# imazen/imageflow

Hardware: AMD Instinct MI355X
Metric: megapixels/sec resize (4K->200px Robidoux) (higher is better)
Workload: dtype f32; 1 GPU; BASELINE cfg2: 256 frames (256 on rank 0) 3840x2160 BGRA8 -> 200x200 Robidoux, linear light, ReplaceSelf, alpha not meaningful, device resident, pattern=mixed; frames_per_gpu=256, total_frames=256, kernel=fused_resample_kernel, gather=none, gather_mode=none, reserved_cus_while_gathering=0, rccl_ranks=1, backend=none

## Files before the change

### imageflow_amd/csrc/api.cpp

```cpp
#include <hip/hip_runtime.h>

#include <algorithm>
#include <cstdio>
#include <cstring>
#include <map>
#include <memory>
#include <mutex>
#include <tuple>
#include <vector>

#include "hip_entry.hpp"
#include "resample_plan.hpp"

namespace ifhip {
hipError_t launch_fused(const ResampleArgs& a, int slots, bool alpha, bool per_pixel, uint32_t grid, uint32_t block,
                        size_t lds, hipStream_t st);
hipError_t launch_generic(const ResampleArgs& a, bool alpha, float4* scratch, uint32_t img0, uint32_t n_img,
                          hipStream_t st);
hipError_t launch_banded(const ResampleArgs& a, bool alpha, const BandedArgs& b, uint32_t grid_x, size_t lds, hipStream_t st);
hipError_t launch_apply_matte(uint8_t* d_bgra, size_t image_bytes, uint32_t n_images, uint32_t w, uint32_t h,
                              uint32_t stride, uint32_t matte, float mb, float mg, float mr, float ma,
                              const float* s2l, const uint8_t* l2s, hipStream_t st);
}

using namespace ifhip;

namespace {
struct DeviceTables {
    float* s2l = nullptr;
    float* s2f = nullptr;
    uint8_t* l2s = nullptr;
    uint16_t* l2s_thr = nullptr;
};
std::mutex g_dev_mu;
std::map<int, DeviceTables> g_dev_tables;

int device_tables(DeviceTables* out) {
    int dev = -1;
    if (hipGetDevice(&dev) != hipSuccess || dev < 0)
        return fail(IFHIP_GPU_UNAVAILABLE, "GpuUnavailable: no HIP device (hipGetDevice failed); this library has no CPU path");
    std::lock_guard<std::mutex> lk(g_dev_mu);
    auto it = g_dev_tables.find(dev);
    if (it == g_dev_tables.end()) {
        hipDeviceProp_t prop;
        HIP_TRY(hipGetDeviceProperties(&prop, dev));
        if (std::strncmp(prop.gcnArchName, "gfx950", 6) != 0)
            return fail(IFHIP_GPU_UNAVAILABLE, "GpuUnavailable: device %d is %s, this library is built for gfx950 only", dev, prop.gcnArchName);
        const ColorTables& t = color_tables();
        DeviceTables d;
        HIP_TRY(hipMalloc(reinterpret_cast<void**>(&d.s2l), sizeof t.s2l));
        HIP_TRY(hipMalloc(reinterpret_cast<void**>(&d.s2f), sizeof t.s2f));
        HIP_TRY(hipMalloc(reinterpret_cast<void**>(&d.l2s), sizeof t.l2s));
        HIP_TRY(hipMemcpy(d.s2l, t.s2l, sizeof t.s2l, hipMemcpyHostToDevice));
        HIP_TRY(hipMemcpy(d.s2f, t.s2f, sizeof t.s2f, hipMemcpyHostToDevice));
        HIP_TRY(hipMemcpy(d.l2s, t.l2s, sizeof t.l2s, hipMemcpyHostToDevice));
        HIP_TRY(hipMalloc(reinterpret_cast<void**>(&d.l2s_thr), sizeof t.l2s_thr));
        HIP_TRY(hipMemcpy(d.l2s_thr, t.l2s_thr, sizeof t.l2s_thr, hipMemcpyHostToDevice));
        it = g_dev_tables.emplace(dev, d).first;
    }
    *out = it->second;
    return IFHIP_OK;
}

template <typename T>
int upload(const std::vector<T>& v, T** out) {
    *out = nullptr;
    if (v.empty()) return IFHIP_OK;
    HIP_TRY(DEV_MALLOC(out, v.size() * sizeof(T)));
    HIP_TRY(static_cast<hipError_t>(copy_to_device(*out, v.data(), v.size() * sizeof(T))));
    return IFHIP_OK;
}

}

struct ifhip_resample_plan {
    int device = -1;
    PlanTables t;
    uint32_t *d_v_left = nullptr, *d_v_count = nullptr, *d_v_off = nullptr;
    uint32_t *d_h_left = nullptr, *d_h_count = nullptr, *d_h_off = nullptr;
    float *d_v_w = nullptr, *d_h_w = nullptr, *d_h_wu = nullptr, *d_h_wg = nullptr, *d_h_wg2 = nullptr;
    uint4* d_h_meta = nullptr;
    uint32_t *d_h_meta2 = nullptr, *d_h_meta3 = nullptr;
    Strip* d_strips[2] = {nullptr, nullptr};

    ~ifhip_resample_plan() {
        for (void* p : {(void*)d_v_left, (void*)d_v_count, (void*)d_v_off, (void*)d_h_left, (void*)d_h_count,
                        (void*)d_h_off, (void*)d_v_w, (void*)d_h_w, (void*)d_h_wu, (void*)d_h_meta, (void*)d_h_wg, (void*)d_h_meta2, (void*)d_h_wg2, (void*)d_h_meta3, (void*)d_strips[0],
                        (void*)d_strips[1]})
            if (p) (void)DEV_FREE(p);
        for (auto& kv : t.schedules) {
            if (kv.second.d_steps) (void)DEV_FREE(kv.second.d_steps);
            if (kv.second.d_band_begin) (void)DEV_FREE(kv.second.d_band_begin);
        }
    }
};

namespace {

bool trace_launch() { return debug_switch("trace_launch") != nullptr; }

int schedule_on_device(const PlanTables& t, PlannedSchedule* s) {
    std::lock_guard<std::mutex> lk(t.mu);
    if (s->d_steps) return IFHIP_OK;
    VStep* steps = nullptr;
    int rc = upload(s->host.steps, &steps);
    if (rc) return rc;
    rc = upload(s->host.band_begin, &s->d_band_begin);
    if (rc) { (void)DEV_FREE(steps); return rc; }
    s->d_steps = steps;
    return IFHIP_OK;
}

int validate_render(uint32_t in_w, uint32_t in_h, uint32_t in_stride, uint32_t cw, uint32_t ch, uint32_t c_stride,
                    uint32_t x, uint32_t y, uint32_t w, uint32_t h, int working_space, int compositing, uint32_t in_px_bytes = 4) {
    if (static_cast<uint64_t>(h) + y > ch || static_cast<uint64_t>(w) + x > cw)
        return fail(IFHIP_INVALID_ARGUMENT, "InvalidArgument: Destination rectangle for scale2d is out of bounds");
    if (w == 0 || h == 0 || in_w == 0 || in_h == 0)
        return fail(IFHIP_INVALID_ARGUMENT, "InvalidArgument: Bitmap dimensions cannot be zero");
    if (static_cast<uint64_t>(in_w) * in_px_bytes > in_stride || static_cast<uint64_t>(cw) * 4u > c_stride)
        return fail(IFHIP_INVALID_ARGUMENT, "InvalidArgument: stride smaller than a BGRA row");
    if (c_stride & 3u)
        return fail(IFHIP_INVALID_ARGUMENT, "InvalidArgument: canvas stride must be a multiple of 4 bytes");
    if (working_space != IFHIP_SPACE_SRGB && working_space != IFHIP_SPACE_LINEAR)
        return fail(IFHIP_METHOD_NOT_IMPLEMENTED, "MethodNotImplemented: working floatspace %d", working_space);
    if (compositing < IFHIP_REPLACE_SELF || compositing > IFHIP_BLEND_WITH_MATTE)
        return fail(IFHIP_INVALID_ARGUMENT, "InvalidArgument: compositing mode %d", compositing);
    return IFHIP_OK;
}

int enqueue_batch(const ifhip_resample_plan* p, const uint8_t* d_in, size_t in_image_bytes, uint32_t in_stride,
                  int alpha, uint32_t n_images, uint8_t* d_canvas, size_t canvas_image_bytes, uint32_t cw, uint32_t ch,
                  uint32_t c_stride, uint32_t x, uint32_t y, int working_space, int compositing, uint32_t matte,
                  float* d_f32, int force_kernel, hipStream_t st, const uint8_t* d_cb = nullptr, const uint8_t* d_cr = nullptr,
                  bool probe = false) {
    if (!p) return fail(IFHIP_INVALID_ARGUMENT, "InvalidArgument: null plan");
    const PlanTables& t = p->t;
    const bool ycc = d_cb != nullptr;
    int rc = validate_render(t.in_w, t.in_h, in_stride, cw, ch, c_stride, x, y, t.out_w, t.out_h, working_space, compositing, ycc ? 1u : 4u);
    if (rc) return rc;
    if (n_images == 0) return IFHIP_OK;
    if (!d_in || !d_canvas || (ycc && !d_cr)) return fail(IFHIP_INVALID_ARGUMENT, "InvalidArgument: null bitmap pointer");
    if ((reinterpret_cast<uintptr_t>(d_canvas) & 3u) || (canvas_image_bytes & 3u))
        return fail(IFHIP_INVALID_ARGUMENT, "InvalidArgument: canvas pixels must be 4-byte aligned");
    int dev = -1;
    HIP_TRY(hipGetDevice(&dev));
    if (dev != p->device) return fail(IFHIP_INVALID_STATE, "InvalidState: plan belongs to device %d, current device is %d", p->device, dev);
    DeviceTables tb;
    rc = device_tables(&tb);
    if (rc) return rc;

    LaunchInputs in = launch_inputs_now();
    in.alpha = alpha; in.ycc = ycc; in.n_images = n_images; in.in_image_bytes = in_image_bytes; in.in_stride = in_stride;
    in.src_low_bits = (reinterpret_cast<uintptr_t>(d_in) | reinterpret_cast<uintptr_t>(d_cb) | reinterpret_cast<uintptr_t>(d_cr)) & 15u;
    in.force_kernel = force_kernel; in.working_space = working_space; in.probe = probe;
    const LaunchChoice c = choose_launch(t, in);
    if (c.status) return c.status;
    if (trace_launch()) std::fprintf(stderr, "%s\n", format_launch(t, in, c).c_str());
    if (probe) return IFHIP_OK;

    const ColorTables& host_tb = color_tables();
    ResampleArgs a;
    std::memset(&a, 0, sizeof a);
    a.in = d_in; a.in_image_bytes = in_image_bytes; a.in_stride = in_stride; a.in_w = t.in_w; a.in_h = t.in_h;
    a.in_cb = d_cb; a.in_cr = d_cr; a.ycc = ycc ? 1u : 0u;
    a.canvas = d_canvas; a.canvas_image_bytes = canvas_image_bytes; a.c_stride = c_stride; a.x = x; a.y = y;
    a.out_w = t.out_w; a.out_h = t.out_h; a.f32_dump = d_f32;
    a.h_meta = p->d_h_meta; a.h_wu = p->d_h_wu; a.h_wu_floats = static_cast<uint32_t>(t.wu.size());
    a.h_left = p->d_h_left; a.h_count = p->d_h_count;
    a.v_left = p->d_v_left; a.v_count = p->d_v_count; a.v_off = p->d_v_off; a.v_w = p->d_v_w;
    a.h_off = p->d_h_off; a.h_w = p->d_h_w;
    a.linear = working_space == IFHIP_SPACE_LINEAR;
    a.lut_in = a.linear ? tb.s2l : tb.s2f;
    a.l2s = tb.l2s;
    a.l2s_thr = tb.l2s_thr;
    a.mode = compositing;
    const float* s2 = a.linear ? host_tb.s2l : host_tb.s2f;
    a.m0 = s2[matte & 255u]; a.m1 = s2[(matte >> 8) & 255u]; a.m2 = s2[(matte >> 16) & 255u];
    a.matte_a = static_cast<float>(matte >> 24) * (1.0f / 255.0f);
    a.n_images = n_images;

    if (c.kernel == LaunchKernel::Banded) {
        HIP_TRY(launch_banded(a, alpha != 0, c.banded, c.grid, c.lds, st));
        return IFHIP_OK;
    }
    if (c.kernel == LaunchKernel::Fused) {
        if ((rc = schedule_on_device(t, c.schedule))) return rc;
        a.steps = c.schedule->d_steps; a.band_begin = c.schedule->d_band_begin; a.n_bands = c.n_bands;
        a.strips = p->d_strips[alpha ? 1 : 0]; a.n_strips = c.n_strips;
        a.h_groups = c.two_col ? 16u + c.fast_groups : c.fast_groups;
        if (c.two_col) { a.h_wu = p->d_h_wg2; a.h_wu_floats = static_cast<uint32_t>(t.wg2.size()); a.h_meta2 = p->d_h_meta3; }
        else if (c.fast_groups) { a.h_wu = p->d_h_wg; a.h_wu_floats = static_cast<uint32_t>(t.wg.size()); a.h_meta2 = p->d_h_meta2; }
        a.lut_copies_log2 = c.lut_copies_log2;
        a.h_w_in_lds = c.w_in_lds ? 1u : 0u;
        a.l2s_in_lds = c.l2s_in_lds ? 1u : 0u;
        a.frames_per_wg = c.frames_per_wg;
        a.lanes_per_frame = c.lanes_per_frame;
        HIP_TRY(launch_fused(a, t.slots, alpha != 0, c.per_pixel, c.grid, c.lanes_per_frame * c.frames_per_wg, c.lds, st));
        return IFHIP_OK;
    }
    const size_t per_image = static_cast<size_t>(t.out_h) * t.in_w * sizeof(float4);
    float4* scratch = nullptr;
    HIP_TRY(static_cast<hipError_t>(cached_malloc_for_stream(reinterpret_cast<void**>(&scratch), per_image * c.chunk, st, true)));
    hipError_t le = hipSuccess;
    for (uint32_t i0 = 0; i0 < n_images && le == hipSuccess; i0 += c.chunk) {
        const uint32_t n = std::min(c.chunk, n_images - i0);
        le = launch_generic(a, alpha != 0, scratch, i0, n, st);
    }
    const hipError_t fe = static_cast<hipError_t>(cached_free_after(scratch, st));
    HIP_TRY(le);
    HIP_TRY(fe);
    return IFHIP_OK;
}
}

namespace ifhip {
int resample_from_ycc_planes_v(const ifhip_resample_plan* plan, const uint8_t* d_y, const uint8_t* d_cb, const uint8_t* d_cr,
                             size_t plane_bytes, uint32_t pitch, uint32_t n_images, uint8_t* d_canvas, size_t canvas_image_bytes,
                             uint32_t cw, uint32_t ch, uint32_t c_stride, uint32_t x, uint32_t y, int working_space, int compositing,
                             uint32_t matte, void* hip_stream, bool probe) {
    return enqueue_batch(plan, d_y, plane_bytes, pitch, 0, n_images, d_canvas, canvas_image_bytes, cw, ch, c_stride, x, y,
                         working_space, compositing, matte, nullptr, -1, static_cast<hipStream_t>(hip_stream), d_cb, d_cr, probe);
}
void resample_plan_shape(const ifhip_resample_plan* plan, uint32_t* in_w, uint32_t* in_h, uint32_t* out_w, uint32_t* out_h) {
    *in_w = plan->t.in_w; *in_h = plan->t.in_h; *out_w = plan->t.out_w; *out_h = plan->t.out_h;
}
int device_color_tables(const float** s2l, const uint8_t** l2s) {
    DeviceTables tb;
    const int rc = device_tables(&tb);
    if (rc) return rc;
    *s2l = tb.s2l; *l2s = tb.l2s;
    return IFHIP_OK;
}

namespace {
struct PlanKey {
    int device; uint32_t in_w, in_h, w, h; int filter; uint32_t sharpen_bits;
    bool operator<(const PlanKey& o) const {
        return std::tie(device, in_w, in_h, w, h, filter, sharpen_bits) < std::tie(o.device, o.in_w, o.in_h, o.w, o.h, o.filter, o.sharpen_bits);
    }
};
std::mutex g_plan_mu;
typedef std::map<PlanKey, std::pair<std::shared_ptr<ifhip_resample_plan>, uint64_t>> PlanMap;
PlanMap& plan_map() { static PlanMap* m = new PlanMap; return *m; }
uint64_t g_plan_clock = 0;
constexpr size_t kPlanCacheMax = 256;
}
int cached_plan(uint32_t in_w, uint32_t in_h, uint32_t w, uint32_t h, int filter, float sharpen, std::shared_ptr<ifhip_resample_plan>* out) {
    int dev = -1;
    if (hipGetDevice(&dev) != hipSuccess || dev < 0)
        return fail(IFHIP_GPU_UNAVAILABLE, "GpuUnavailable: no HIP device (hipGetDevice failed); this library has no CPU path");
    uint32_t bits;
    std::memcpy(&bits, &sharpen, 4);
    const PlanKey key{dev, in_w, in_h, w, h, filter, bits};
    {
        std::lock_guard<std::mutex> lk(g_plan_mu);
        auto it = plan_map().find(key);
        if (it != plan_map().end()) { it->second.second = ++g_plan_clock; *out = it->second.first; return IFHIP_OK; }
    }
    ifhip_resample_plan* raw = nullptr;
    const int rc = ifhip_resample_plan_create(&raw, in_w, in_h, w, h, filter, sharpen);
    if (rc) return rc;
    std::shared_ptr<ifhip_resample_plan> sp(raw, [](ifhip_resample_plan* q) {
        if (hipStream_t st = static_cast<hipStream_t>(thread_stream()); st && hipStreamQuery(st) != hipSuccess) (void)wait_stream(st);
        (void)hipGetLastError();
        ifhip_resample_plan_destroy(q);
    });
    std::shared_ptr<ifhip_resample_plan> evicted;
    {
        std::lock_guard<std::mutex> lk(g_plan_mu);
        PlanMap& plans = plan_map();
// ... 307 lines not shown
```

### imageflow_amd/csrc/common.hpp

```cpp
#pragma once
#include <cstdint>
#include <memory>
#include <string>
#include <vector>

#include "../../include/imageflow_hip.h"

namespace ifhip {

int fail(int status, const char* fmt, ...) __attribute__((format(printf, 2, 3)));
const char* last_error();

int cached_malloc(void** out, size_t bytes);
int cached_free(void* p);
int cached_malloc_for_stream(void** out, size_t bytes, void* stream, bool for_stream);
int cached_free_after(void* p, void* stream);
int cached_host_malloc(void** out, size_t bytes);
int cached_host_free(void* p);
void quiesced_enter();
void quiesced_leave();
struct QuiescedScope { QuiescedScope() { quiesced_enter(); } ~QuiescedScope() { quiesced_leave(); } };
void* thread_stream();
int wait_stream(void* hip_stream);
int copy_to_device(void* dst, const void* src, size_t bytes);
int stage_to_device(void* dst, const void* src, size_t bytes, void** pin_out);
int copy_to_host(void* dst, const void* src, size_t bytes);
int zero_device(void* dst, size_t bytes);
int require_gfx950(int* device_out);
#define DEV_MALLOC(pp, n) static_cast<hipError_t>(::ifhip::cached_malloc(reinterpret_cast<void**>(pp), (n)))
#define DEV_FREE(p) static_cast<hipError_t>(::ifhip::cached_free(p))

bool icc_describes_srgb(const uint8_t* profile, size_t profile_bytes);
int jpeg_icc_profile(const uint8_t* jpeg, size_t len, int* kind, std::vector<uint8_t>* profile);

const char* debug_switch(const char* key);
inline bool debug_on(const char* key) { return debug_switch(key) != nullptr; }

enum class KernelShape : uint8_t { FlexCubic, CubicFast, Sinc, Box, Triangle, SincWindowed, Jinc, Ginseng };

struct FilterSpec {
    double window = 2.0;
    double blur = 1.0;
    double p1 = 0, p2 = 1, p3 = 1, q1 = 0, q2 = 1, q3 = 1, q4 = 1;
    KernelShape shape = KernelShape::Box;
    int lobe_mode = IFHIP_LOBE_NATURAL;
    float lobe_value = 0.f;

    double eval(double x) const;
    double natural_negative_ratio() const;
};

bool filter_spec_for(int filter, FilterSpec* out);

struct AxisWeights {
    uint32_t n_out = 0, n_in = 0;
    std::vector<uint32_t> left;
    std::vector<uint32_t> count;
    std::vector<uint32_t> offset;
    std::vector<float> w;
    uint32_t max_taps = 0;
};

int build_axis_weights(const FilterSpec& spec, uint32_t out_size, uint32_t in_size, AxisWeights* out);

struct ColorTables {
    float s2l[256];
    float s2f[256];
    uint8_t l2s[16384];
    uint16_t l2s_thr[256];
};
const ColorTables& color_tables();
int device_color_tables(const float** s2l, const uint8_t** l2s);

constexpr int kMaxSlots = 8;
struct alignas(64) VStep {
    int32_t y;
    uint32_t active;
    int32_t flush_slot;
    int32_t out_row;
    float w[kMaxSlots];
    int32_t y_ahead;
    int32_t pad[3];
};
static_assert(sizeof(VStep) == 64, "VStep must be one 64-byte scalar-load line");

struct VSchedule {
    int slots = 0;
    std::vector<VStep> steps;
    std::vector<uint32_t> band_begin;
};
bool build_vschedule(const AxisWeights& wv, int n_bands, int group, int ahead, VSchedule* out);

constexpr int kNotFusable = -1000;
int resample_from_ycc_planes_v(const ifhip_resample_plan* plan, const uint8_t* d_y, const uint8_t* d_cb, const uint8_t* d_cr,
                               size_t plane_bytes, uint32_t pitch, uint32_t n_images, uint8_t* d_canvas, size_t canvas_image_bytes,
                               uint32_t cw, uint32_t ch, uint32_t c_stride, uint32_t x, uint32_t y, int working_space, int compositing,
                               uint32_t matte, void* hip_stream, bool probe = false);
void resample_plan_shape(const ifhip_resample_plan* plan, uint32_t* in_w, uint32_t* in_h, uint32_t* out_w, uint32_t* out_h);
int max_live_rows(const AxisWeights& wv);
int cached_plan(uint32_t in_w, uint32_t in_h, uint32_t w, uint32_t h, int filter, float sharpen, std::shared_ptr<ifhip_resample_plan>* out);

}
```

### imageflow_amd/csrc/resample_fused.hip

```cpp
#include <atomic>
#include <type_traits>

#include "resample_device.hpp"

#ifndef IFHIP_FUSED_K
#error "compile with -DIFHIP_FUSED_K=<ring size 1..8>"
#endif
namespace ifhip {

template <int K, bool ALPHA, bool WLDS, bool PERPIXEL, int FG = 0, bool YCC = false>
__global__ void __launch_bounds__(fused_max_threads(K, ALPHA ? 4 : 3))
__attribute__((amdgpu_waves_per_eu(fused_max_threads(K, ALPHA ? 4 : 3) / 256, fused_max_threads(K, ALPHA ? 4 : 3) / 256)))
fused_resample_kernel(const ResampleArgs a, const VStep* __restrict__ steps) {
    static_assert(FG == 0 || (WLDS && PERPIXEL), "the fast horizontal pass keeps its weights in LDS and maps one lane per pixel");
    constexpr bool TWO = FG >= 16;
    static_assert(!TWO || (!ALPHA && !YCC), "two-column groups: three channels from a BGRA source");
    static_assert(!YCC || (!ALPHA && fused_shape(K, 3).px == 4), "planar source: three channels, four pixels per lane");
    constexpr int C = ALPHA ? 4 : 3;
    constexpr int D = fused_shape(K, C).rows_in_flight;
    constexpr bool PIPE = fused_shape(K, C).pipelined != 0;
    extern __shared__ __attribute__((aligned(16))) unsigned char smem[];

    const uint32_t wtid = threadIdx.x;
    const uint32_t WT = blockDim.x;
    const uint32_t T = a.lanes_per_frame;
    const uint32_t slot = __builtin_amdgcn_readfirstlane(wtid / T);
    const uint32_t tid = wtid - slot * T;
    uint32_t b = blockIdx.x;
    if (a.n_strips > 1u && (gridDim.x & 7u) == 0u) b = (b & 7u) * (gridDim.x >> 3) + (b >> 3);
    const uint32_t strip_i = b % a.n_strips; b /= a.n_strips;
    const uint32_t band = b % a.n_bands;
    const uint32_t img_raw = (b / a.n_bands) * a.frames_per_wg + slot;
    const bool img_on = img_raw < a.n_images;
    const uint32_t img = img_on ? img_raw : a.n_images - 1u;

    const Strip strip = a.strips[strip_i];
    const uint32_t n_u = strip.u1 - strip.u0;

    constexpr uint32_t fast_g = TWO ? FG - 16 : FG;
    constexpr uint32_t GP = fused_group_pitch(C);
    const FusedLds L = fused_lds_layout(n_u, strip.nquads, a.h_wu_floats, C, WLDS, a.l2s_in_lds != 0, a.lut_copies_log2, PERPIXEL,
                                        a.frames_per_wg, fast_g);
    float* lut_banked = reinterpret_cast<float*>(smem + L.lut);
    uint16_t* thr = reinterpret_cast<uint16_t*>(smem + L.thr);
    uint4* hmeta = reinterpret_cast<uint4*>(smem + L.hmeta);
    float* obuf = reinterpret_cast<float*>(smem + L.obuf + slot * L.obuf_stride);
    const float* hw_lds = reinterpret_cast<const float*>(smem + L.hw);
    float* inter = reinterpret_cast<float*>(smem + L.inter + slot * 2u * L.inter_stride);
    const uint32_t inter_stride = L.inter_stride >> 2;
    const uint32_t plane_pitch = L.plane_pitch;
    const uint32_t obuf_stride = n_u * 4u;

    for (uint32_t i = wtid; i < (256u << a.lut_copies_log2); i += WT) lut_banked[i] = a.lut_in[i >> a.lut_copies_log2];
    for (uint32_t i = wtid; i < 256u; i += WT) thr[i] = a.l2s_thr[i];
    const uint8_t* l2s_lds = a.l2s_in_lds ? smem + L.l2s : nullptr;
    if (a.l2s_in_lds)
        for (uint32_t i = wtid; i < 1024u; i += WT)
            reinterpret_cast<uint4*>(smem + L.l2s)[i] = reinterpret_cast<const uint4*>(a.l2s)[i];
    const BankedLut lut{lut_banked, wtid & ((1u << a.lut_copies_log2) - 1u), a.lut_copies_log2};
    uint32_t* hmeta2 = reinterpret_cast<uint32_t*>(smem + L.hmeta);
    if constexpr (FG > 0) {
        for (uint32_t i = wtid; i < n_u; i += WT) hmeta2[i] = a.h_meta2[strip.u0 + i] - (strip.cx0 >> (TWO ? 1 : 2));
        float4* z = reinterpret_cast<float4*>(smem + L.inter);
        for (uint32_t i = wtid; i < (a.frames_per_wg * 2u * L.inter_stride) >> 4; i += WT) z[i] = make_float4(0.f, 0.f, 0.f, 0.f);
    } else {
        for (uint32_t i = wtid; i < n_u; i += WT) {
            uint4 m = a.h_meta[strip.u0 + i];
            m.x -= strip.cx0;
            hmeta[i] = m;
        }
    }
    if (WLDS) {
        const float4* src4 = reinterpret_cast<const float4*>(a.h_wu);
        float4* dst4 = reinterpret_cast<float4*>(smem + L.hw);
        for (uint32_t i = wtid; i < (a.h_wu_floats >> 2); i += WT) dst4[i] = src4[i];
    }
    __syncthreads();
    auto lds_barrier = [] {
        __builtin_amdgcn_fence(__ATOMIC_RELEASE, "workgroup", "local");
        __builtin_amdgcn_s_barrier();
        __builtin_amdgcn_fence(__ATOMIC_ACQUIRE, "workgroup", "local");
    };

    const uint32_t s0 = a.band_begin[band], s1 = a.band_begin[band + 1];
    constexpr int PX = fused_shape(K, C).px;
    const uint32_t n_groups = strip.nquads * (4u / PX);
    const bool lane_on = tid < n_groups;
    const uint32_t quad = lane_on ? tid : n_groups - 1u;
    constexpr uint32_t BPP = YCC ? 1u : 4u;
    const uint32_t img_u = __builtin_amdgcn_readfirstlane(img);
    const uint8_t* src = a.in + (static_cast<size_t>(img_u) * a.in_image_bytes + static_cast<size_t>(strip.cx0) * BPP);
    const uint32_t lane_off0 = static_cast<uint32_t>(PX) * quad * BPP;

    typedef float f32x2 __attribute__((ext_vector_type(2)));
    typedef float f32x4 __attribute__((ext_vector_type(4)));
    constexpr int NP = PX * C / 2;
    f32x2 acc[K][NP];
#pragma unroll
    for (int s = 0; s < K; ++s)
#pragma unroll
        for (int i = 0; i < NP; ++i) acc[s][i] = f32x2{0.0f, 0.0f};
    auto acc_at = [&](int s, int p, int c) -> float {
        const int f = p * C + c;
        return (f & 1) ? acc[s][f >> 1].y : acc[s][f >> 1].x;
    };

    typedef uint32_t bgra_raw_t __attribute__((ext_vector_type(PX)));
    struct YccRaw { uint32_t y, cb, cr; };
    typedef std::conditional_t<YCC, YccRaw, bgra_raw_t> raw_t;
    auto fetch_row = [&](int y) -> raw_t {
        const uint32_t yy = y < 0 ? 0u : static_cast<uint32_t>(y);
        uint64_t rowp = reinterpret_cast<uint64_t>(src) + static_cast<uint64_t>(yy) * a.in_stride;
        asm("" : "+s"(rowp));
        uint32_t lane_off = lane_off0;
        asm("" : "+v"(lane_off));
        typedef __attribute__((address_space(1))) const uint8_t gbyte;
        typedef __attribute__((address_space(1))) const uint32_t gword;
        typedef __attribute__((address_space(1))) const bgra_raw_t graw;
        gbyte* py = reinterpret_cast<gbyte*>(rowp);
        if constexpr (YCC) {
            return YccRaw{__builtin_nontemporal_load(reinterpret_cast<gword*>(py + lane_off)),
                          __builtin_nontemporal_load(reinterpret_cast<gword*>(py + (a.in_cb - a.in) + lane_off)),
                          __builtin_nontemporal_load(reinterpret_cast<gword*>(py + (a.in_cr - a.in) + lane_off))};
        } else {
            return __builtin_nontemporal_load(reinterpret_cast<graw*>(py + lane_off));
        }
    };

    const uint32_t lut_mul = 4u << a.lut_copies_log2;
    typedef __attribute__((address_space(3))) const float lds_cfloat;
    typedef __attribute__((address_space(3))) unsigned char lds_byte;
    const uint32_t lut_lane = static_cast<uint32_t>(reinterpret_cast<uintptr_t>((lds_byte*)(smem + L.lut))) + (lut.lane_off << 2);
    auto convert = [&](const raw_t& q, f32x2 (&vv)[NP]) {
        float v[PX][C];
        if constexpr (YCC) {
            uint32_t ad[PX][3];
#pragma unroll
            for (int p = 0; p < PX; ++p) {
                const int32_t Y = static_cast<int32_t>((q.y >> (8 * p)) & 255u);
                const int32_t cb = static_cast<int32_t>((q.cb >> (8 * p)) & 255u) - 128, cr = static_cast<int32_t>((q.cr >> (8 * p)) & 255u) - 128;
                const int32_t r = Y + ((__mul24(91881, cr) + 32768) >> 16);
                const int32_t g = Y + ((__mul24(-22554, cb) + 32768 + __mul24(-46802, cr)) >> 16);
                const int32_t b = Y + ((__mul24(116130, cb) + 32768) >> 16);
                const int32_t ch[3] = {b, g, r};
#pragma unroll
                for (int k = 0; k < 3; ++k) {
                    const int32_t c8 = ch[k] < 0 ? 0 : (ch[k] > 255 ? 255 : ch[k]);
                    ad[p][k] = __umul24(static_cast<uint32_t>(c8), lut_mul) + lut_lane;
                }
            }
            __builtin_amdgcn_sched_barrier(0);
#pragma unroll
            for (int p = 0; p < PX; ++p)
#pragma unroll
                for (int k = 0; k < 3; ++k) v[p][k] = *reinterpret_cast<lds_cfloat*>(static_cast<uintptr_t>(ad[p][k]));
        } else {
        uint32_t ad[PX][3];
#pragma unroll
        for (int p = 0; p < PX; ++p)
#pragma unroll
            for (int k = 0; k < 3; ++k) ad[p][k] = __builtin_amdgcn_udot4(q[p], lut_mul << (8 * k), lut_lane, false);
        __builtin_amdgcn_sched_barrier(0);
#pragma unroll
        for (int p = 0; p < PX; ++p) {
            const uint32_t px = q[p];
#pragma unroll
            for (int k = 0; k < 3; ++k) v[p][k] = *reinterpret_cast<lds_cfloat*>(static_cast<uintptr_t>(ad[p][k]));
            if (ALPHA) {
                const float af = static_cast<float>(px >> 24) * (1.0f / 255.0f);
                v[p][0] = v[p][0] * af;
                v[p][1] = v[p][1] * af;
                v[p][2] = v[p][2] * af;
                v[p][C - 1] = af;
            }
        }
        }
#pragma unroll
        for (int i = 0; i < NP; ++i) vv[i] = f32x2{v[(2 * i) / C][(2 * i) % C], v[(2 * i + 1) / C][(2 * i + 1) % C]};
    };

    auto h_pair_group = [&](f32x2& h, const float4& w, const float4& t01, const float4& t23) {
        h = __builtin_elementwise_fma(f32x2{w.x, w.x}, f32x2{t01.x, t01.y}, h);
        h = __builtin_elementwise_fma(f32x2{w.y, w.y}, f32x2{t01.z, t01.w}, h);
        h = __builtin_elementwise_fma(f32x2{w.z, w.z}, f32x2{t23.x, t23.y}, h);
        h = __builtin_elementwise_fma(f32x2{w.w, w.w}, f32x2{t23.z, t23.w}, h);
    };
    auto h_single_group = [&](float& h, const float4& w, const float4& t) {
        h = __builtin_fmaf(w.x, t.x, h);
        h = __builtin_fmaf(w.y, t.y, h);
        h = __builtin_fmaf(w.z, t.z, h);
        h = __builtin_fmaf(w.w, t.w, h);
    };
    const uint32_t n_chain = n_u * 2u;
    const uint32_t n_store = img_on ? n_u : 0u;
    auto h_run_row = [&](const float* vrow, float* orow) {
        for (uint32_t idx = tid; idx < n_chain; idx += T) {
            const uint32_t ul = idx >> 1, g = idx & 1u;
            const uint4 m = hmeta[ul];
            const float4* wp = reinterpret_cast<const float4*>((WLDS ? hw_lds : a.h_wu) + m.z);
            if (g == 0u || ALPHA) {
                const float4* s0 = reinterpret_cast<const float4*>(vrow + (2u * g) * plane_pitch + m.x);
                const float4* s1 = reinterpret_cast<const float4*>(vrow + (2u * g + 1u) * plane_pitch + m.x);
                f32x2 h = {0.0f, 0.0f};
                for (uint32_t q = 0; q < m.y; ++q) h_pair_group(h, wp[q], s0[q], s1[q]);
                *reinterpret_cast<float2*>(orow + ul * 4u + 2u * g) = make_float2(h.x, h.y);
            } else {
                const float4* sp = reinterpret_cast<const float4*>(vrow + 2u * plane_pitch + m.x);
                float h = 0.0f;
                for (uint32_t q = 0; q < m.y; ++q) h_single_group(h, wp[q], sp[q]);
                orow[ul * 4u + 2u] = h;
            }
        }
    };
    uint32_t tid_h = tid;
    if constexpr (PERPIXEL) {
        const uint32_t q = (tid >> 2) & 7u;
        const uint32_t first4 = (0x7326'1540u >> (4u * q)) & 15u;
        tid_h = (tid & ~31u) | (first4 << 2) | (tid & 3u);
    }
    constexpr bool h_per_pixel = PERPIXEL;
    auto h_run_row_pixels = [&](uint32_t j, const float* vrow) {
        for (uint32_t ul = tid_h; ul < n_store; ul += T) {
            const uint4 m = hmeta[ul];
            const float4* wp = reinterpret_cast<const float4*>((WLDS ? hw_lds : a.h_wu) + m.z);
            const float4* sp = reinterpret_cast<const float4*>(vrow + m.x);
            const uint32_t pp4 = plane_pitch >> 2;
            f32x2 h01 = {0.0f, 0.0f}, h23 = {0.0f, 0.0f};
            float h2 = 0.0f;
            constexpr int HPU = fused_shape(K, C).threads == 512 ? 2 : 1;
#pragma unroll HPU
            for (uint32_t q = 0; q < m.y; ++q) {
                const float4 w = wp[q];
                h_pair_group(h01, w, sp[q], sp[pp4 + q]);
                if (ALPHA) h_pair_group(h23, w, sp[2u * pp4 + q], sp[3u * pp4 + q]);
                else h_single_group(h2, w, sp[2u * pp4 + q]);
            }
            const OutTables<BankedLut, ThresholdL2S> tb{lut, ThresholdL2S{thr, l2s_lds}};
            store_pixel<ALPHA>(a, img, j, strip.u0 + ul, h01.x, h01.y, ALPHA ? h23.x : h2, ALPHA ? h23.y : 1.0f, tb);
        }
    };
    auto h_run_row_pixels_fast = [&](uint32_t j, const float* vrow, auto static_encode) {
        constexpr uint32_t G = fast_g > 0 ? fast_g : 1;
        for (uint32_t ul = tid_h; ul < n_store; ul += T) {
            const uint32_t m = hmeta2[ul];
            f32x2 h01 = {0.0f, 0.0f}, h23 = {0.0f, 0.0f};
            float h2 = 0.0f;
            if constexpr (TWO) {
                typedef __attribute__((address_space(3))) const f32x2 lds_f2;
                uint32_t a0 = static_cast<uint32_t>(reinterpret_cast<uintptr_t>((lds_byte*)(reinterpret_cast<const unsigned char*>(vrow)))) + (m & 0xffffu) * (GP / 2u);
                uint32_t a1 = a0 + 8u, a2 = a0 + 16u;
                asm volatile("" : "+v"(a0), "+v"(a1), "+v"(a2));
                const float2* wp = reinterpret_cast<const float2*>(hw_lds) + (m >> 16) * G;
#pragma unroll
                for (uint32_t q = 0; q < G; ++q) {
                    const float2 w = wp[q];
                    const f32x2 t0 = *reinterpret_cast<lds_f2*>(static_cast<uintptr_t>(a0 + q * (GP / 2u)));
                    const f32x2 t1 = *reinterpret_cast<lds_f2*>(static_cast<uintptr_t>(a1 + q * (GP / 2u)));
                    const f32x2 c2 = *reinterpret_cast<lds_f2*>(static_cast<uintptr_t>(a2 + q * (GP / 2u)));
                    h01 = __builtin_elementwise_fma(f32x2{w.x, w.x}, f32x2{t0.x, t0.y}, h01);
                    h01 = __builtin_elementwise_fma(f32x2{w.y, w.y}, f32x2{t1.x, t1.y}, h01);
                    h2 = __builtin_fmaf(w.x, c2.x, h2);
                    h2 = __builtin_fmaf(w.y, c2.y, h2);
                    asm volatile("" : "+v"(h01));
                    asm volatile("" : "+v"(h2));
                    __builtin_amdgcn_sched_barrier(0);
                }
            } else {
            const unsigned char* sp = reinterpret_cast<const unsigned char*>(vrow) + (m & 0xffffu) * GP;
            const float4* wp = reinterpret_cast<const float4*>(hw_lds) + (m >> 16) * G;
#pragma unroll
            for (uint32_t q = 0; q < G; ++q) {
                const float4* g = reinterpret_cast<const float4*>(sp + q * GP);
                const float4 w = wp[q];
                h_pair_group(h01, w, g[0], g[1]);
                if (ALPHA) h_pair_group(h23, w, g[2], g[3]);
                else h_single_group(h2, w, g[2]);
                asm volatile("" : "+v"(h01));
                if (ALPHA) asm volatile("" : "+v"(h23));
                else asm volatile("" : "+v"(h2));
                __builtin_amdgcn_sched_barrier(0);
            }
            }
            if constexpr (decltype(static_encode)::value) {
                const OutTables<BankedLut, DirectL2S> tbs{lut, DirectL2S{l2s_lds}};
                store_pixel<ALPHA, 1>(a, img, j, strip.u0 + ul, h01.x, h01.y, ALPHA ? h23.x : h2, ALPHA ? h23.y : 1.0f, tbs);
            } else {
                const OutTables<BankedLut, ThresholdL2S> tb{lut, ThresholdL2S{thr, l2s_lds}};
                store_pixel<ALPHA>(a, img, j, strip.u0 + ul, h01.x, h01.y, ALPHA ? h23.x : h2, ALPHA ? h23.y : 1.0f, tb);
            }
        }
    };
    int h_out_row = -1;
    auto h_store_row = [&](uint32_t j, const float* orow) {
        for (uint32_t ul = T - 1u - tid; ul < n_store; ul += T) {
            const float4 o = *reinterpret_cast<const float4*>(orow + ul * 4u);
            const OutTables<BankedLut, ThresholdL2S> tb{lut, ThresholdL2S{thr, l2s_lds}};
            store_pixel<ALPHA>(a, img, j, strip.u0 + ul, o.x, o.y, o.z, ALPHA ? o.w : 1.0f, tb);
        }
    };

    raw_t raw[D];
#pragma unroll
    for (int d = 0; d < D; ++d) {
        raw[d] = fetch_row(steps[s0 + d].y);
        __builtin_amdgcn_sched_barrier(0);
    }
    f32x2 vbuf[PIPE ? 2 : 1][NP];
    VStep rec[PIPE ? 2 : 1];
    if (PIPE) {
        rec[0] = steps[s0];
        convert(raw[0], vbuf[0]);
        __builtin_amdgcn_sched_barrier(0);
        raw[0] = fetch_row((s0 + D < s1) ? steps[s0 + D].y : -1);
        __builtin_amdgcn_sched_barrier(0);
    }

    for (uint32_t sb = s0; sb < s1; sb += D) {
#pragma unroll
        for (int d = 0; d < D; ++d) {
            const int cur = PIPE ? (d & 1) : 0, nxt = PIPE ? (cur ^ 1) : 0;
            const uint32_t si = sb + d;
            if (PIPE) {
                const int slot_next = (d + 1) % D;
                rec[nxt] = steps[(si + 1 < s1) ? si + 1 : si];
                convert(raw[slot_next], vbuf[nxt]);
                __builtin_amdgcn_sched_barrier(0);
                raw[slot_next] = fetch_row(rec[cur].y_ahead);
                __builtin_amdgcn_sched_barrier(0);
            } else {
                rec[0] = steps[si];
                convert(raw[d], vbuf[0]);
                __builtin_amdgcn_sched_barrier(0);
                raw[d] = fetch_row(rec[0].y_ahead);
                __builtin_amdgcn_sched_barrier(0);
            }
            const VStep& st = rec[cur];
            f32x2 (&v)[NP] = vbuf[PIPE ? cur : 0];
            if (st.y >= 0) {
#pragma unroll
                for (int s = 0; s < K; ++s) {
                    const float w = st.w[s];
#pragma unroll
                    for (int i = 0; i < NP; ++i) acc[s][i] = __builtin_elementwise_fma(f32x2{w, w}, v[i], acc[s][i]);
                }
            }
            if (st.flush_slot >= 0) {
                const uint32_t j = static_cast<uint32_t>(st.out_row);
                float* dst_row = inter + (j & 1u) * inter_stride;
#pragma unroll
                for (int s = 0; s < K; ++s) {
                    if (st.flush_slot == s) {
                        if (lane_on) {
                            const uint32_t pp4 = plane_pitch >> 2;
                            if constexpr (FG > 0) {
                                static_assert(FG == 0 || PX == 4, "fast pass: 4 source pixels per lane");
                                float4* g4 = reinterpret_cast<float4*>(reinterpret_cast<unsigned char*>(dst_row) + tid * GP);
                                if constexpr (TWO) {
                                    g4[0] = make_float4(acc_at(s, 0, 0), acc_at(s, 0, 1), acc_at(s, 1, 0), acc_at(s, 1, 1));
                                    g4[1] = make_float4(acc_at(s, 0, 2), acc_at(s, 1, 2), acc_at(s, 2, 0), acc_at(s, 2, 1));
                                    g4[2] = make_float4(acc_at(s, 3, 0), acc_at(s, 3, 1), acc_at(s, 2, 2), acc_at(s, 3, 2));
                                } else {
                                    g4[0] = make_float4(acc_at(s, 0, 0), acc_at(s, 0, 1), acc_at(s, 1, 0), acc_at(s, 1, 1));
                                    g4[1] = make_float4(acc_at(s, 2, 0), acc_at(s, 2, 1), acc_at(s, 3, 0), acc_at(s, 3, 1));
                                    if (ALPHA) {
                                        g4[2] = make_float4(acc_at(s, 0, 2), acc_at(s, 0, C - 1), acc_at(s, 1, 2), acc_at(s, 1, C - 1));
                                        g4[3] = make_float4(acc_at(s, 2, 2), acc_at(s, 2, C - 1), acc_at(s, 3, 2), acc_at(s, 3, C - 1));
                                    } else {
                                        g4[2] = make_float4(acc_at(s, 0, 2), acc_at(s, 1, 2), acc_at(s, 2, 2), acc_at(s, 3, 2));
                                    }
                                }
                            } else if constexpr (PX == 4) {
                                float4* g4 = reinterpret_cast<float4*>(dst_row + 4u * tid);
                                g4[0] = make_float4(acc_at(s, 0, 0), acc_at(s, 0, 1), acc_at(s, 1, 0), acc_at(s, 1, 1));
                                g4[pp4] = make_float4(acc_at(s, 2, 0), acc_at(s, 2, 1), acc_at(s, 3, 0), acc_at(s, 3, 1));
                                if (ALPHA) {
                                    g4[2u * pp4] = make_float4(acc_at(s, 0, 2), acc_at(s, 0, C - 1), acc_at(s, 1, 2), acc_at(s, 1, C - 1));
                                    g4[3u * pp4] = make_float4(acc_at(s, 2, 2), acc_at(s, 2, C - 1), acc_at(s, 3, 2), acc_at(s, 3, C - 1));
                                } else {
                                    g4[2u * pp4] = make_float4(acc_at(s, 0, 2), acc_at(s, 1, 2), acc_at(s, 2, 2), acc_at(s, 3, 2));
                                }
                            } else {
                                const uint32_t half = tid & 1u;
                                float4* g4 = reinterpret_cast<float4*>(dst_row + 4u * (tid >> 1));
                                g4[half * pp4] = make_float4(acc_at(s, 0, 0), acc_at(s, 0, 1), acc_at(s, 1, 0), acc_at(s, 1, 1));
                                if (ALPHA) g4[(2u + half) * pp4] = make_float4(acc_at(s, 0, 2), acc_at(s, 0, C - 1), acc_at(s, 1, 2), acc_at(s, 1, C - 1));
                                else *reinterpret_cast<float2*>(dst_row + 2u * plane_pitch + 2u * tid) = make_float2(acc_at(s, 0, 2), acc_at(s, 1, 2));
                            }
                        }
#pragma unroll
                        for (int i = 0; i < NP; ++i) acc[s][i] = f32x2{0.0f, 0.0f};
                    }
                }
                lds_barrier();
                if constexpr (h_per_pixel) {
                    if constexpr (FG > 0) {
                        if (a.linear && l2s_lds != nullptr) h_run_row_pixels_fast(j, dst_row, std::true_type{});
                        else h_run_row_pixels_fast(j, dst_row, std::false_type{});
                    }
                    else h_run_row_pixels(j, dst_row);
                } else {
                    if (h_out_row >= 0) h_store_row(static_cast<uint32_t>(h_out_row), obuf + (static_cast<uint32_t>(h_out_row) & 1u) * obuf_stride);
                    h_out_row = static_cast<int>(j);
                    h_run_row(dst_row, obuf + (j & 1u) * obuf_stride);
                }
            }
        }
    }
    if (h_out_row >= 0) {
        lds_barrier();
        h_store_row(static_cast<uint32_t>(h_out_row), obuf + (static_cast<uint32_t>(h_out_row) & 1u) * obuf_stride);
    }
}


template <int K, bool ALPHA, bool WLDS, bool PERPIXEL, int FG = 0, bool YCC = false>
static hipError_t launch_variant(const ResampleArgs& a, dim3 grid, dim3 block, size_t lds, hipStream_t st) {
    static std::atomic<uint64_t> raised;
    int dev = 0;
    hipError_t e = hipGetDevice(&dev);
    if (e != hipSuccess) return e;
    const uint64_t bit = dev >= 0 && dev < 64 ? 1ull << dev : 0ull;
    if (!(raised.load(std::memory_order_relaxed) & bit)) {
        e = hipFuncSetAttribute(reinterpret_cast<const void*>(&fused_resample_kernel<K, ALPHA, WLDS, PERPIXEL, FG, YCC>),
                                hipFuncAttributeMaxDynamicSharedMemorySize, static_cast<int>(kFusedLdsCap));
        if (e != hipSuccess) return e;
        raised.fetch_or(bit, std::memory_order_relaxed);
// ... 60 lines not shown
```

### imageflow_amd/csrc/resample_plan.hpp

```cpp
#pragma once
#include <hip/hip_vector_types.h>

#include <map>
#include <mutex>
#include <string>
#include <vector>

#include "device.hpp"

namespace ifhip {

constexpr uint32_t kComputeUnits = 256;
void set_cu_budget(uint32_t compute_units);

struct PlannedSchedule {
    VSchedule host;
    VStep* d_steps = nullptr;
    uint32_t* d_band_begin = nullptr;
};

struct PlanTables {
    uint32_t in_w = 0, in_h = 0, out_w = 0, out_h = 0;
    AxisWeights wv, wh;
    std::vector<float> wu;
    std::vector<uint4> hmeta;
    uint32_t h_avg_groups = 0;
    uint32_t h_fast_groups = 0;
    std::vector<float> wg;
    std::vector<uint32_t> hmeta2;
    uint32_t h_two_groups = 0;
    std::vector<float> wg2;
    std::vector<uint32_t> hmeta3;
    bool fused_possible = false;
    int slots = 0;
    struct StripSet {
        std::vector<Strip> strips;
        uint32_t max_quads = 0;
        bool ok = false;
    } sets[2];
    mutable std::mutex mu;
    mutable std::map<uint64_t, PlannedSchedule> schedules;
};
int resample_filter_spec(int filter, float sharpen_percent_goal, FilterSpec* out);
int build_plan_tables(uint32_t in_w, uint32_t in_h, uint32_t w, uint32_t h, const FilterSpec& spec, PlanTables* out);

struct LaunchInputs {
    int alpha = 0;
    bool ycc = false;
    uint32_t n_images = 0;
    size_t in_image_bytes = 0;
    uint32_t in_stride = 0;
    uintptr_t src_low_bits = 0;
    int force_kernel = -1;
    int working_space = IFHIP_SPACE_LINEAR;
    bool probe = false;
    uint32_t cu_budget = 0;
    uint32_t banded_wgs = 0, banded_strip = 0, banded_flags = 0xffffffffu;
};
LaunchInputs launch_inputs_now();

enum class LaunchKernel { Fused, Banded, Generic };
struct LaunchChoice {
    int status = IFHIP_OK;
    LaunchKernel kernel = LaunchKernel::Generic;
    uint32_t grid = 0;
    size_t lds = 0;
    uint32_t lanes_per_frame = 0, frames_per_wg = 1, n_strips = 0;
    bool per_pixel = false;
    uint32_t fast_groups = 0;
    bool two_col = false;
    bool w_in_lds = false, l2s_in_lds = false;
    uint32_t lut_copies_log2 = 0;
    uint32_t want_bands = 0, n_bands = 0;
    PlannedSchedule* schedule = nullptr;
    BandedArgs banded{};
    uint32_t instead_of_fused_lanes = 0;
    uint32_t chunk = 0;
};
LaunchChoice choose_launch(const PlanTables& t, const LaunchInputs& in);
std::string format_launch(const PlanTables& t, const LaunchInputs& in, const LaunchChoice& c);

}
```

### imageflow_amd/csrc/weights.cpp

```cpp
#include <cmath>
#include <cstdarg>
#include <cstdio>
#include <cstring>
#include <atomic>
#include <map>
#include <mutex>

#include "common.hpp"

namespace ifhip {

static thread_local char g_err[512] = "";

int fail(int status, const char* fmt, ...) {
    va_list ap;
    va_start(ap, fmt);
    vsnprintf(g_err, sizeof g_err, fmt, ap);
    va_end(ap);
    return status;
}
const char* last_error() { return g_err; }

namespace {
std::atomic<int> g_switches_set{0};
// ... 218 lines not shown
                    scale_neg = static_cast<float>(want_neg / sum_neg);
                }
            } else if (sum == 0.0) {
                return fail(IFHIP_INVALID_STATE, "InvalidState: TotalWeightZero at output %u (%u -> %u)", u, in_size, out_size);
            }
        }
        for (uint32_t i = 0; i < n; ++i) taps[i] *= (taps[i] < 0.f) ? scale_neg : scale_pos;

        uint32_t b = 0, e = n;
        while (e > b && taps[e - 1] == 0.f) --e;
        while (b < e && taps[b] == 0.f) ++b;
        if (e == b)
            return fail(IFHIP_INVALID_STATE, "InvalidState: NoPixelInputs at output %u (%u -> %u)", u, in_size, out_size);
        r.left[u] = first + b;
        r.count[u] = e - b;
        r.offset[u] = static_cast<uint32_t>(r.w.size());
        r.w.insert(r.w.end(), taps.begin() + b, taps.begin() + e);
        if (e - b > r.max_taps) r.max_taps = e - b;
    }
    *out = std::move(r);
    return IFHIP_OK;
}

int max_live_rows(const AxisWeights& wv) {
    int best = 0;
    uint32_t lo = 0;
    for (uint32_t j = 0; j < wv.n_out; ++j) {
        while (lo < j && wv.left[lo] + wv.count[lo] - 1 < wv.left[j]) ++lo;
        const int live = static_cast<int>(j - lo + 1);
        if (live > best) best = live;
    }
    return best;
}

bool build_vschedule(const AxisWeights& wv, int n_bands, int group, int ahead, VSchedule* out) {
    if (group < 1 || ahead < 1) return false;
    const int K = max_live_rows(wv);
    if (K > kMaxSlots) return false;
    for (uint32_t j = 1; j < wv.n_out; ++j) {
        if (wv.left[j] < wv.left[j - 1]) return false;
        if (wv.left[j] + wv.count[j] < wv.left[j - 1] + wv.count[j - 1]) return false;
    }
    if (n_bands < 1) n_bands = 1;
    if (static_cast<uint32_t>(n_bands) > wv.n_out) n_bands = static_cast<int>(wv.n_out);
    VSchedule s;
    s.slots = K;
    s.band_begin.push_back(0);
    for (int b = 0; b < n_bands; ++b) {
        const uint32_t j0 = static_cast<uint32_t>(static_cast<uint64_t>(wv.n_out) * b / n_bands);
        const uint32_t j1 = static_cast<uint32_t>(static_cast<uint64_t>(wv.n_out) * (b + 1) / n_bands);
        const uint32_t y0 = wv.left[j0];
        const uint32_t y1 = wv.left[j1 - 1] + wv.count[j1 - 1] - 1;
        uint32_t jlo = j0;
        for (uint32_t y = y0; y <= y1; ++y) {
            VStep st;
            std::memset(&st, 0, sizeof st);
            st.y = static_cast<int32_t>(y);
            st.flush_slot = -1; st.out_row = -1;
            bool any = false;
            std::vector<uint32_t> done;
            for (uint32_t j = jlo; j < j1 && wv.left[j] <= y; ++j) {
                const uint32_t last = wv.left[j] + wv.count[j] - 1;
                if (y > last) continue;
                const int slot = static_cast<int>(j % K);
                st.active |= 1u << slot;
                st.w[slot] = wv.w[wv.offset[j] + (y - wv.left[j])];
                any = true;
                if (y == last) done.push_back(j);
            }
            if (!any && done.empty()) continue;
            if (!done.empty()) { st.flush_slot = static_cast<int32_t>(done[0] % K); st.out_row = static_cast<int32_t>(done[0]); }
            s.steps.push_back(st);
            for (size_t i = 1; i < done.size(); ++i) {
                VStep f;
                std::memset(&f, 0, sizeof f);
                f.y = -1; f.flush_slot = static_cast<int32_t>(done[i] % K); f.out_row = static_cast<int32_t>(done[i]);
                s.steps.push_back(f);
            }
            while (jlo < j1 && wv.left[jlo] + wv.count[jlo] - 1 <= y) ++jlo;
        }
        while ((s.steps.size() - s.band_begin.back()) % static_cast<size_t>(group) != 0) {
            VStep nop;
            std::memset(&nop, 0, sizeof nop);
            nop.y = -1; nop.flush_slot = -1; nop.out_row = -1; nop.y_ahead = -1;
            s.steps.push_back(nop);
        }
        const size_t begin = s.band_begin.back(), end = s.steps.size();
        for (size_t i = begin; i < end; ++i) {
            const size_t a = i + static_cast<size_t>(ahead);
            s.steps[i].y_ahead = a < end ? s.steps[a].y : -1;
        }
        s.band_begin.push_back(static_cast<uint32_t>(s.steps.size()));
    }
    *out = std::move(s);
    return true;
}

}

extern "C" int ifhip_debug_set(const char* key, const char* value) {
    if (!key || !*key) return ifhip::fail(IFHIP_INVALID_ARGUMENT, "InvalidArgument: null switch name");
    std::lock_guard<std::mutex> lk(ifhip::g_switch_mu);
    ifhip::switches()[key] = value ? new std::string(value) : nullptr;
    ifhip::g_switches_set.store(1, std::memory_order_relaxed);
    return IFHIP_OK;
}
```

Before: 1.600 million MP/s.

## Precompute refill byte offsets per stride and tighten fused vertical step loop

Step records now carry a precomputed 64-bit refill byte offset, uploaded once per input stride, so the kernel no longer multiplies row by stride or clamps negative rows on every fetch. The step loop walks a scalar pointer with a sentinel record instead of indexing, drops the y>=0 branch, and issues packed FMAs with scalar weight pairs through inline asm. The horizontal pass with weights in LDS uses explicit LDS addresses that advance by a fixed increment. Costs are more device memory (one schedule copy per stride) and FMAs that now also run on no-op steps, which rely on those steps having zero weights.

```diff
diff --git a/imageflow_amd/csrc/api.cpp b/imageflow_amd/csrc/api.cpp
--- a/imageflow_amd/csrc/api.cpp
+++ b/imageflow_amd/csrc/api.cpp
@@ -89,7 +89,7 @@
                         (void*)d_strips[1]})
             if (p) (void)DEV_FREE(p);
         for (auto& kv : t.schedules) {
-            if (kv.second.d_steps) (void)DEV_FREE(kv.second.d_steps);
+            for (auto& ds : kv.second.d_steps) (void)DEV_FREE(ds.second);
             if (kv.second.d_band_begin) (void)DEV_FREE(kv.second.d_band_begin);
         }
     }
@@ -99,15 +99,17 @@
 
 bool trace_launch() { return debug_switch("trace_launch") != nullptr; }
 
-int schedule_on_device(const PlanTables& t, PlannedSchedule* s) {
+int schedule_on_device(const PlanTables& t, PlannedSchedule* s, uint32_t stride, const VStep** d_steps) {
     std::lock_guard<std::mutex> lk(t.mu);
-    if (s->d_steps) return IFHIP_OK;
-    VStep* steps = nullptr;
-    int rc = upload(s->host.steps, &steps);
-    if (rc) return rc;
-    rc = upload(s->host.band_begin, &s->d_band_begin);
-    if (rc) { (void)DEV_FREE(steps); return rc; }
-    s->d_steps = steps;
+    auto it = s->d_steps.find(stride);
+    if (it == s->d_steps.end()) {
+        VStep* steps = nullptr;
+        int rc = upload(steps_for_stride(s->host, stride), &steps);
+        if (rc) return rc;
+        if (!s->d_band_begin && (rc = upload(s->host.band_begin, &s->d_band_begin))) { (void)DEV_FREE(steps); return rc; }
+        it = s->d_steps.emplace(stride, steps).first;
+    }
+    *d_steps = it->second;
     return IFHIP_OK;
 }
 
@@ -184,8 +186,8 @@
         return IFHIP_OK;
     }
     if (c.kernel == LaunchKernel::Fused) {
-        if ((rc = schedule_on_device(t, c.schedule))) return rc;
-        a.steps = c.schedule->d_steps; a.band_begin = c.schedule->d_band_begin; a.n_bands = c.n_bands;
+        if ((rc = schedule_on_device(t, c.schedule, in_stride, &a.steps))) return rc;
+        a.band_begin = c.schedule->d_band_begin; a.n_bands = c.n_bands;
         a.strips = p->d_strips[alpha ? 1 : 0]; a.n_strips = c.n_strips;
         a.h_groups = c.two_col ? 16u + c.fast_groups : c.fast_groups;
         if (c.two_col) { a.h_wu = p->d_h_wg2; a.h_wu_floats = static_cast<uint32_t>(t.wg2.size()); a.h_meta2 = p->d_h_meta3; }
diff --git a/imageflow_amd/csrc/common.hpp b/imageflow_amd/csrc/common.hpp
--- a/imageflow_amd/csrc/common.hpp
+++ b/imageflow_amd/csrc/common.hpp
@@ -74,13 +74,14 @@
 
 constexpr int kMaxSlots = 8;
 struct alignas(64) VStep {
+    int32_t flush_slot;
+    int32_t out_row;
+    uint64_t refill_off;
+    float w[kMaxSlots];
     int32_t y;
     uint32_t active;
-    int32_t flush_slot;
-    int32_t out_row;
-    float w[kMaxSlots];
-    int32_t y_ahead;
-    int32_t pad[3];
+    int32_t refill_row;
+    int32_t pad;
 };
 static_assert(sizeof(VStep) == 64, "VStep must be one 64-byte scalar-load line");
 
@@ -90,6 +91,7 @@
     std::vector<uint32_t> band_begin;
 };
 bool build_vschedule(const AxisWeights& wv, int n_bands, int group, int ahead, VSchedule* out);
+std::vector<VStep> steps_for_stride(const VSchedule& s, uint32_t stride);
 
 constexpr int kNotFusable = -1000;
 int resample_from_ycc_planes_v(const ifhip_resample_plan* plan, const uint8_t* d_y, const uint8_t* d_cb, const uint8_t* d_cr,
diff --git a/imageflow_amd/csrc/resample_fused.hip b/imageflow_amd/csrc/resample_fused.hip
--- a/imageflow_amd/csrc/resample_fused.hip
+++ b/imageflow_amd/csrc/resample_fused.hip
@@ -90,7 +90,7 @@
     constexpr uint32_t BPP = YCC ? 1u : 4u;
     const uint32_t img_u = __builtin_amdgcn_readfirstlane(img);
     const uint8_t* src = a.in + (static_cast<size_t>(img_u) * a.in_image_bytes + static_cast<size_t>(strip.cx0) * BPP);
-    const uint32_t lane_off0 = static_cast<uint32_t>(PX) * quad * BPP;
+    uint32_t lane_off0 = static_cast<uint32_t>(PX) * quad * BPP;
 
     typedef float f32x2 __attribute__((ext_vector_type(2)));
     typedef float f32x4 __attribute__((ext_vector_type(4)));
@@ -108,12 +108,11 @@
     typedef uint32_t bgra_raw_t __attribute__((ext_vector_type(PX)));
     struct YccRaw { uint32_t y, cb, cr; };
     typedef std::conditional_t<YCC, YccRaw, bgra_raw_t> raw_t;
-    auto fetch_row = [&](int y) -> raw_t {
-        const uint32_t yy = y < 0 ? 0u : static_cast<uint32_t>(y);
-        uint64_t rowp = reinterpret_cast<uint64_t>(src) + static_cast<uint64_t>(yy) * a.in_stride;
+    auto fetch_row = [&](uint64_t row_off) -> raw_t {
+        uint64_t rowp = reinterpret_cast<uint64_t>(src) + row_off;
         asm("" : "+s"(rowp));
-        uint32_t lane_off = lane_off0;
-        asm("" : "+v"(lane_off));
+        asm("" : "+v"(lane_off0));
+        const uint32_t lane_off = lane_off0;
         typedef __attribute__((address_space(1))) const uint8_t gbyte;
         typedef __attribute__((address_space(1))) const uint32_t gword;
         typedef __attribute__((address_space(1))) const bgra_raw_t graw;
@@ -179,13 +178,13 @@
         for (int i = 0; i < NP; ++i) vv[i] = f32x2{v[(2 * i) / C][(2 * i) % C], v[(2 * i + 1) / C][(2 * i + 1) % C]};
     };
 
-    auto h_pair_group = [&](f32x2& h, const float4& w, const float4& t01, const float4& t23) {
+    auto h_pair_group = [&](f32x2& h, const auto& w, const auto& t01, const auto& t23) {
         h = __builtin_elementwise_fma(f32x2{w.x, w.x}, f32x2{t01.x, t01.y}, h);
         h = __builtin_elementwise_fma(f32x2{w.y, w.y}, f32x2{t01.z, t01.w}, h);
         h = __builtin_elementwise_fma(f32x2{w.z, w.z}, f32x2{t23.x, t23.y}, h);
         h = __builtin_elementwise_fma(f32x2{w.w, w.w}, f32x2{t23.z, t23.w}, h);
     };
-    auto h_single_group = [&](float& h, const float4& w, const float4& t) {
+    auto h_single_group = [&](float& h, const auto& w, const auto& t) {
         h = __builtin_fmaf(w.x, t.x, h);
         h = __builtin_fmaf(w.y, t.y, h);
         h = __builtin_fmaf(w.z, t.z, h);
@@ -222,18 +221,36 @@
     auto h_run_row_pixels = [&](uint32_t j, const float* vrow) {
         for (uint32_t ul = tid_h; ul < n_store; ul += T) {
             const uint4 m = hmeta[ul];
-            const float4* wp = reinterpret_cast<const float4*>((WLDS ? hw_lds : a.h_wu) + m.z);
-            const float4* sp = reinterpret_cast<const float4*>(vrow + m.x);
-            const uint32_t pp4 = plane_pitch >> 2;
             f32x2 h01 = {0.0f, 0.0f}, h23 = {0.0f, 0.0f};
             float h2 = 0.0f;
             constexpr int HPU = fused_shape(K, C).threads == 512 ? 2 : 1;
+            if constexpr (WLDS) {
+                typedef __attribute__((address_space(3))) const f32x4 lds_f4;
+                auto lds_addr = [](const void* p) { return static_cast<uint32_t>(reinterpret_cast<uintptr_t>((lds_byte*)(reinterpret_cast<const unsigned char*>(p)))); };
+                auto ld = [](uint32_t ad) -> f32x4 { return *reinterpret_cast<lds_f4*>(static_cast<uintptr_t>(ad)); };
+                const uint32_t pp = plane_pitch << 2;
+                uint32_t aw = lds_addr(hw_lds) + (m.z << 2), a0 = lds_addr(vrow) + (m.x << 2), a1 = a0 + pp, a2 = a1 + pp, a3 = a2 + pp;
+                asm volatile("" : "+v"(aw), "+v"(a0), "+v"(a1), "+v"(a2), "+v"(a3));
+#pragma unroll HPU
+                for (uint32_t q = m.y; q != 0u; --q) {
+                    const f32x4 w = ld(aw);
+                    h_pair_group(h01, w, ld(a0), ld(a1));
+                    if (ALPHA) h_pair_group(h23, w, ld(a2), ld(a3));
+                    else h_single_group(h2, w, ld(a2));
+                    aw += 16u; a0 += 16u; a1 += 16u; a2 += 16u;
+                    if (ALPHA) a3 += 16u;
+                }
+            } else {
+            const float4* wp = reinterpret_cast<const float4*>(a.h_wu + m.z);
+            const float4* sp = reinterpret_cast<const float4*>(vrow + m.x);
+            const uint32_t pp4 = plane_pitch >> 2;
 #pragma unroll HPU
             for (uint32_t q = 0; q < m.y; ++q) {
                 const float4 w = wp[q];
                 h_pair_group(h01, w, sp[q], sp[pp4 + q]);
                 if (ALPHA) h_pair_group(h23, w, sp[2u * pp4 + q], sp[3u * pp4 + q]);
                 else h_single_group(h2, w, sp[2u * pp4 + q]);
+            }
             }
             const OutTables<BankedLut, ThresholdL2S> tb{lut, ThresholdL2S{thr, l2s_lds}};
             store_pixel<ALPHA>(a, img, j, strip.u0 + ul, h01.x, h01.y, ALPHA ? h23.x : h2, ALPHA ? h23.y : 1.0f, tb);
@@ -299,49 +316,67 @@
         }
     };
 
+    struct StepRec { int32_t flush_slot, out_row; uint64_t refill_off; float w[K]; };
+    typedef __attribute__((address_space(4))) const unsigned char crec_byte;
+    typedef __attribute__((address_space(4))) const VStep crec;
+    static_assert(offsetof(VStep, flush_slot) == 0 && offsetof(VStep, out_row) == 4 && offsetof(VStep, refill_off) == 8 &&
+                  offsetof(VStep, w) == 16, "what a step reads is the head of its record");
+    crec_byte* sp = reinterpret_cast<crec_byte*>(reinterpret_cast<uintptr_t>(steps + s0));
+    crec_byte* const sp_end = reinterpret_cast<crec_byte*>(reinterpret_cast<uintptr_t>(steps + s1));
+    auto load_rec = [](crec_byte* p) -> StepRec {
+        crec* q = reinterpret_cast<crec*>(p);
+        StepRec r;
+        r.flush_slot = q->flush_slot; r.out_row = q->out_row; r.refill_off = q->refill_off;
+#pragma unroll
+        for (int s = 0; s < K; ++s) r.w[s] = q->w[s];
+        return r;
+    };
+    auto row_off_of = [&](int y) -> uint64_t { return static_cast<uint64_t>(y < 0 ? 0 : y) * a.in_stride; };
+
     raw_t raw[D];
 #pragma unroll
     for (int d = 0; d < D; ++d) {
-        raw[d] = fetch_row(steps[s0 + d].y);
+        raw[d] = fetch_row(row_off_of(steps[s0 + d].y));
         __builtin_amdgcn_sched_barrier(0);
     }
     f32x2 vbuf[PIPE ? 2 : 1][NP];
-    VStep rec[PIPE ? 2 : 1];
+    StepRec rec[PIPE ? 2 : 1];
     if (PIPE) {
-        rec[0] = steps[s0];
+        rec[0] = load_rec(sp);
         convert(raw[0], vbuf[0]);
         __builtin_amdgcn_sched_barrier(0);
-        raw[0] = fetch_row((s0 + D < s1) ? steps[s0 + D].y : -1);
+        raw[0] = fetch_row(row_off_of((s0 + D < s1) ? steps[s0 + D].y : -1));
         __builtin_amdgcn_sched_barrier(0);
     }
 
-    for (uint32_t sb = s0; sb < s1; sb += D) {
+    for (; sp != sp_end; sp += D * sizeof(VStep)) {
 #pragma unroll
         for (int d = 0; d < D; ++d) {
             const int cur = PIPE ? (d & 1) : 0, nxt = PIPE ? (cur ^ 1) : 0;
-            const uint32_t si = sb + d;
             if (PIPE) {
                 const int slot_next = (d + 1) % D;
-                rec[nxt] = steps[(si + 1 < s1) ? si + 1 : si];
+                rec[nxt] = load_rec(sp + (d + 1) * sizeof(VStep));
                 convert(raw[slot_next], vbuf[nxt]);
                 __builtin_amdgcn_sched_barrier(0);
-                raw[slot_next] = fetch_row(rec[cur].y_ahead);
+                raw[slot_next] = fetch_row(rec[cur].refill_off);
                 __builtin_amdgcn_sched_barrier(0);
             } else {
-                rec[0] = steps[si];
+                rec[0] = load_rec(sp + d * sizeof(VStep));
                 convert(raw[d], vbuf[0]);
                 __builtin_amdgcn_sched_barrier(0);
-                raw[d] = fetch_row(rec[0].y_ahead);
+                raw[d] = fetch_row(rec[0].refill_off);
                 __builtin_amdgcn_sched_barrier(0);
             }
-            const VStep& st = rec[cur];
+            const StepRec& st = rec[cur];
             f32x2 (&v)[NP] = vbuf[PIPE ? cur : 0];
-            if (st.y >= 0) {
-#pragma unroll
-                for (int s = 0; s < K; ++s) {
-                    const float w = st.w[s];
-#pragma unroll
-                    for (int i = 0; i < NP; ++i) acc[s][i] = __builtin_elementwise_fma(f32x2{w, w}, v[i], acc[s][i]);
+#pragma unroll
+            for (int s = 0; s < K; s += 2) {
+                const f32x2 wp = {st.w[s], st.w[s + 1 < K ? s + 1 : s]};
+#pragma unroll
+                for (int i = 0; i < NP; ++i) asm("v_pk_fma_f32 %0, %1, %2, %0 op_sel_hi:[0,1,1]" : "+v"(acc[s][i]) : "s"(wp), "v"(v[i]));
+                if (s + 1 < K) {
+#pragma unroll
+                    for (int i = 0; i < NP; ++i) asm("v_pk_fma_f32 %0, %1, %2, %0 op_sel:[1,0,0]" : "+v"(acc[s + 1][i]) : "s"(wp), "v"(v[i]));
                 }
             }
             if (st.flush_slot >= 0) {
diff --git a/imageflow_amd/csrc/resample_plan.hpp b/imageflow_amd/csrc/resample_plan.hpp
--- a/imageflow_amd/csrc/resample_plan.hpp
+++ b/imageflow_amd/csrc/resample_plan.hpp
@@ -15,7 +15,7 @@
 
 struct PlannedSchedule {
     VSchedule host;
-    VStep* d_steps = nullptr;
+    std::map<uint32_t, VStep*> d_steps;
     uint32_t* d_band_begin = nullptr;
 };
 
diff --git a/imageflow_amd/csrc/weights.cpp b/imageflow_amd/csrc/weights.cpp
--- a/imageflow_amd/csrc/weights.cpp
+++ b/imageflow_amd/csrc/weights.cpp
@@ -324,18 +324,28 @@
         while ((s.steps.size() - s.band_begin.back()) % static_cast<size_t>(group) != 0) {
             VStep nop;
             std::memset(&nop, 0, sizeof nop);
-            nop.y = -1; nop.flush_slot = -1; nop.out_row = -1; nop.y_ahead = -1;
+            nop.y = -1; nop.flush_slot = -1; nop.out_row = -1;
             s.steps.push_back(nop);
         }
         const size_t begin = s.band_begin.back(), end = s.steps.size();
         for (size_t i = begin; i < end; ++i) {
             const size_t a = i + static_cast<size_t>(ahead);
-            s.steps[i].y_ahead = a < end ? s.steps[a].y : -1;
+            s.steps[i].refill_row = a < end && s.steps[a].y > 0 ? s.steps[a].y : 0;
         }
         s.band_begin.push_back(static_cast<uint32_t>(s.steps.size()));
     }
+    VStep sentinel;
+    std::memset(&sentinel, 0, sizeof sentinel);
+    sentinel.y = -1; sentinel.flush_slot = -1; sentinel.out_row = -1;
+    s.steps.push_back(sentinel);
     *out = std::move(s);
     return true;
+}
+
+std::vector<VStep> steps_for_stride(const VSchedule& s, uint32_t stride) {
+    std::vector<VStep> steps = s.steps;
+    for (VStep& st : steps) st.refill_off = static_cast<uint64_t>(static_cast<uint32_t>(st.refill_row)) * stride;
+    return steps;
 }
 
 }
```

Result: no change. 1.589 million MP/s (-0.7%).
